# cavelandiah/BBMap

Hardware: AMD Instinct MI355X
Metric: aligned_reads_per_sec (higher is better)
Workload: dtype int32

## Files before the change

bbmap_amd/csrc/mapper.hip:

```cpp
#include <hip/hip_runtime.h>

#include "index_common.h"
#include "mapper_dev.h"

namespace bbmapper {

template <bool KARG> __device__ __forceinline__ const Dev &dev_of(const Dev &byValue) {
    if (KARG) return *(const Dev *)__builtin_amdgcn_kernarg_segment_ptr();
    return byValue;
}

__device__ inline int imin(int a, int b) { return a < b ? a : b; }
__device__ inline int imax(int a, int b) { return a > b ? a : b; }
__device__ inline int iabsdif(int a, int b) { return a > b ? a - b : b - a; }
__device__ inline int max_quality(const Settings &S, int len) { return S.ptsMatch + (len - 1) * S.ptsMatch2; }
__device__ inline int max_imperfect(const Settings &S, int len) { return max_quality(S, len) + S.impDelta; }

__device__ void fix_gaps2(Site &ss) {
    int ra[BBMSA_MAX_GAPS / 2], rb[BBMSA_MAX_GAPS / 2];
    bool alive[BBMSA_MAX_GAPS / 2];
    const int nr = ss.ngaps / 2;
    for (int i = 0; i < nr; i++) { ra[i] = ss.gaps[2 * i]; rb[i] = ss.gaps[2 * i + 1]; alive[i] = true; }
    for (int i = 1; i < nr; i++)
        if (alive[i - 1] && ra[i] - rb[i - 1] <= MINGAP) { ra[i] = imin(ra[i - 1], ra[i]); rb[i] = imax(rb[i - 1], rb[i]); alive[i - 1] = false; }
// ... 728 lines not shown
        }
    }
    const unsigned long long m = __ballot(stillActive);
    if (m) {
        const int lane = threadIdx.x & 63;
        unsigned base = 0;
        if (lane == __builtin_ctzll(m)) base = atomicAdd(&D.counters[CNT_NEXT_ACTIVE], (unsigned)__builtin_popcountll(m));
        base = __shfl(base, __builtin_ctzll(m));
        if (stillActive) D.activeOut[base + __builtin_popcountll(m & ((1ull << lane) - 1ull))] = (int)r;
    }
}

__global__ __launch_bounds__(128) void finish_kernel(const Dev D) {
    const long long r = (long long)blockIdx.x * blockDim.x + threadIdx.x;
    if (r >= D.nreads) return;
    int n = D.mcount[r];
    if (n <= 0) return;
    Site *s = D.ms + r * D.cap;
    n = merge_duplicate_sites(s, n);
    if (!D.S.paired) sort_sites<false>(s, n);
    D.mcount[r] = n;
}

__global__ __launch_bounds__(128) void rescue_plan_kernel(const Dev D) {
    const long long p = (long long)blockIdx.x * blockDim.x + threadIdx.x;
    if (2 * p + 1 >= D.nreads) return;
    PairResc pr = D.pres[p];
    pr.first = 0; pr.count = 0; pr.ran = 0;
    const long long ra = 2 * p + D.pass, rl = 2 * p + (1 - D.pass);
    int na = D.mcount[ra], nl = D.mcount[rl];
    if (na < 0 || nl < 0) { D.pres[p] = pr; return; }
    Site *sa = D.ms + ra * D.cap;
    const Site *sl = D.ms + rl * D.cap;
    int unpairedA;
    if (D.pass == 0) {
        int u1 = 0, u2 = 0;
        for (int i = 0; i < na; i++) if (sa[i].pairedScore == 0) u1++;
        for (int i = 0; i < nl; i++) if (sl[i].pairedScore == 0) u2++;
        pr.unpaired2 = u2; unpairedA = u1;
    } else unpairedA = pr.unpaired2;
    if (!(unpairedA > 0 && na > 0)) { D.pres[p] = pr; return; }
    pr.ran = 1;
    const int lenA = D.reads[ra].len, L = D.reads[rl].len;
    sort_sites<false>(sa, na);
    na = remove_low_quality_paired(sa, na, max_quality(D.S, lenA), D.S.ratioPreRescue, D.S.ratioPreRescue);
    D.mcount[ra] = na;
    const int searchDist = imin(D.S.maxPairDist, 2 * D.S.averagePairDist + 100);
    if (D.S.rescueSkip || searchDist > D.S.maxRescueDist || na == 0) { D.pres[p] = pr; return; }
    const int maxLooseSw = max_quality(D.S, L), maxAnchorSw = max_quality(D.S, lenA), maxImp = max_imperfect(D.S, L);
    const int bestLoose = nl == 0 ? 0 : sl[0].slowScore, bestAnchor = sa[0].slowScore;
    if (bestLoose == maxLooseSw && bestAnchor == maxAnchorSw && sa[0].pairedScore > 0) { D.pres[p] = pr; return; }
    const int rescueScoreLimit = (int)__fmul_rn(0.95f, (float)bestAnchor);
    pr.retainLimit = imax((int)__fmul_rn(0.68f, (float)bestLoose), (int)__fmul_rn(0.4f, (float)maxLooseSw));
    pr.retainLimit2 = imax((int)__fmul_rn(0.95f, (float)bestLoose), (int)__fmul_rn(0.55f, (float)maxLooseSw));
    pr.maxMismatches = bestLoose > maxImp ? 5 : imin(D.S.maxRescueMismatches, (int)__fsub_rn(__fmul_rn(0.60f, (float)L), 1.0f));
    pr.findTip = (D.S.tipSearchDist > 0 && bestLoose < maxImp) ? 1 : 0;
    int cnt = 0;
    for (int i = 0; i < na; i++) { if (sa[i].slowScore < rescueScoreLimit) break; if (sa[i].pairedScore == 0 && !sa[i].rescued) cnt++; }
    if (cnt == 0) { D.pres[p] = pr; return; }
    const unsigned first = atomicAdd(&D.counters[CNT_RESCUE_SEARCHES], (unsigned)cnt);
    pr.first = (int)first; pr.count = cnt;
    if ((long long)first + cnt <= D.rescCap) {
        const bbidx_read rrl = D.reads[rl];
        int k = 0;
        for (int i = 0; i < na; i++) {
            const Site &ssa = sa[i];
            if (ssa.slowScore < rescueScoreLimit) break;
            if (!(ssa.pairedScore == 0 && !ssa.rescued)) continue;
            const int searchIntoAnchor = ssa.stop - ssa.start - 1 + (lenA * 11 / 16);
            const int strand = ssa.strand ^ 1;
            bbresc_job j;
            j.read_off = rrl.bases_off + (strand ? D.minusDelta : 0);
            j.read_len = L; j.chrom = ssa.chrom;
            if (ssa.strand == 0) { j.loc = ssa.stop - searchIntoAnchor; j.idealStart = ssa.stop + D.S.averagePairDist; }
            else { j.loc = ssa.start + searchIntoAnchor; j.idealStart = ssa.start - D.S.averagePairDist; }
            j.searchDist = searchDist + searchIntoAnchor; j.maxAllowedMismatches = pr.maxMismatches;
            j.flags = strand == 1 ? 1 : 0; j.reserved = 0;
            D.rjobs[first + k] = j;
            RescInfo ri; ri.pair = (int)p; ri.anchorSite = i; ri.strand = strand; ri.job = -1;
            D.rinfo[first + k] = ri;
            k++;
        }
    }
    D.pres[p] = pr;
}

template <bool KARG> __global__ __launch_bounds__(128, 5) void rescue_prep_kernel(const Dev Darg) {
    const Dev &D = dev_of<KARG>(Darg);
    const long long p = (long long)blockIdx.x * blockDim.x + threadIdx.x;
    if (2 * p + 1 >= D.nreads) return;
    const PairResc pr = D.pres[p];
    if (pr.count == 0 || (long long)pr.first + pr.count > D.rescCap) return;
    const long long rl = 2 * p + (1 - D.pass);
    const bbidx_read rrl = D.reads[rl];
    const int L = rrl.len, maxImp = max_imperfect(D.S, L), maxScore = max_quality(D.S, L);
    int seq = D.slow[rl].seq;
    for (int k = 0; k < pr.count; k++) {
        const long long q = pr.first + k;
        RescInfo ri = D.rinfo[q];
        const bbresc_result res = D.rres[q];
        const bbresc_job rj = D.rjobs[q];
        Site ss;
        ss.chrom = rj.chrom; ss.strand = ri.strand; ss.start = res.start; ss.stop = res.stop; ss.hits = 0;
        ss.quickScore = ss.score = res.score; ss.slowScore = 0; ss.pairedScore = 0;
        ss.perfect = res.perfect; ss.semiperfect = res.semiperfect; ss.rescued = 1; ss.ngaps = 0;
        for (int i = 0; i < BBMSA_MAX_GAPS; i++) ss.gaps[i] = 0;
        ss.match_job = -1; ss.reserved[0] = 0; ss.reserved[1] = 0;
        ri.job = -1;
        const int reflen = D.chromArrLen[rj.chrom];
        if (res.found == 1 && ss.start >= 0 && ss.stop <= reflen - 1 && res.mismatches <= pr.maxMismatches) {
            const uint8_t *bases = D.bases + rj.read_off;
            const uint8_t *ref = D.chromArr[rj.chrom];
            int sw = score_no_indels(D.S, bases, L, ref, reflen, ss.start);
            if (sw < maxImp && D.S.maxIndel > 0) {
                set_slow_score(ss, sw);
                if (pr.findTip && find_tip_deletions(D.S, ss, bases, L, ref, reflen, maxImp, true, true)) sw = score_no_indels(D.S, bases, L, ref, reflen, ss.start);
                const int minMsaLimit = -D.S.clearzone1e + (int)__fmul_rn(D.S.ratioPaired, (float)maxScore);
                ri.job = emit_fill(D, rl, rrl, ss, -1, D.S.slowRescuePadding, imax(sw, minMsaLimit), 2, seq++);
                atomicAdd(&D.counters[CNT_RESCUE_FILLS], 1u);
                ss.reserved[0] = 2; ss.reserved[1] = sw;
            } else {
                set_slow_score(ss, sw); ss.score = ss.slowScore; set_stop(ss, ss.start + L - 1);
                ss.reserved[0] = 1; ss.reserved[1] = sw;
            }
        }
        D.rsite[q] = ss;
        D.rinfo[q] = ri;
    }
    D.slow[rl].seq = seq;
}

__global__ __launch_bounds__(128) void rescue_finish_kernel(const Dev D) {
    const long long p = (long long)blockIdx.x * blockDim.x + threadIdx.x;
    if (2 * p + 1 >= D.nreads) return;
    const PairResc pr = D.pres[p];
    if (!pr.ran) return;
    const long long ra = 2 * p + D.pass, rl = 2 * p + (1 - D.pass);
    Site *sa = D.ms + ra * D.cap, *sl = D.ms + rl * D.cap;
    int nl = D.mcount[rl];
    const int nsearch = ((long long)pr.first + pr.count > D.rescCap) ? 0 : pr.count;
    const bbidx_read rrl = D.reads[rl];
    const int L = rrl.len, maxScore = max_quality(D.S, L);
    bool overflow = false;
    for (int k = 0; k < nsearch; k++) {
        const long long q = pr.first + k;
        Site ss = D.rsite[q];
        if (ss.reserved[0] == 0) continue;
        const RescInfo ri = D.rinfo[q];
        const uint8_t *bases = D.bases + D.rjobs[q].read_off;
        const uint8_t *ref = D.chromArr[ss.chrom]; const int reflen = D.chromArrLen[ss.chrom];
        if (ss.reserved[0] == 2) {
            const bbmsa_result &res = fill_result(D, ri.job);
            if (res.score_len > 0) { set_slow_score(ss, res.score[0]); ss.score = ss.slowScore; set_start(ss, res.score[1]); set_stop(ss, res.score[2]); ss.match_job = ri.job; }
            else { const int oldStart = D.rres[q].start; set_slow_score(ss, ss.reserved[1]); ss.score = ss.slowScore; set_start(ss, oldStart); set_stop(ss, ss.start + L - 1); }
        }
        ss.reserved[0] = ss.reserved[1] = 0;
        ss.pairedScore = ss.score + 1;
        ss.perfect = (ss.slowScore == maxScore);
        if (ss.perfect) ss.semiperfect = 1; else set_perfect(D.S, ss, bases, L, ref, reflen);
        if (ss.score > pr.retainLimit && ss.start >= 0 && ss.stop <= reflen - 1) {
// ... 162 lines not shown
```

bbmap_amd/csrc/mapper_ctx.h:

```cpp
#pragma once
#include <hip/hip_runtime.h>

#include <cstdio>
#include <thread>
#include <vector>

#include "bbmap_amd.h"
#include "host_common.h"
#include "index_ctx.h"
#include "mapper_dev.h"
#include "msa_ctx.h"

enum { HIO_READS, HIO_BASES, HIO_SCORES, HIO_KEYINFO, HIO_COUNTS, HIO_OFFSETS, HIO_PACKED, BUF_PACK_TMP, BUF_SAM_TMP, BUF_SAM_TEXT, BUF_COUNT };

enum { ACC_STATS, ACC_COV, ACC_HIST, ACC_SPLIT, ACC_COUNT };
struct Accum { bool counted = false; hipStream_t stream = nullptr; };

struct bbmap_ctx {
    bbmap_config cfg;
    bbidx_ctx *index;
    hipStream_t hostStream = nullptr;
    bbidx_launch probeLs;
    bbmsa_ctx *msa, *msaGapped;
    bbmapper::Settings S;
// ... 6 lines not shown
    unsigned *d_counters;
    bbmsa_job *d_jobs; bbmap_jobinfo *d_jinfo; bbmsa_result *d_results; uint8_t *d_match;
    bbmsa_job *d_gjobs; bbmsa_gaps *d_ggaps; bbmap_jobinfo *d_ginfo; bbmsa_result *d_gresults; uint8_t *d_gmatch;
    bbresc_job *d_rjobs; bbmapper::RescInfo *d_rinfo; bbresc_result *d_rres; bbmapper::PairResc *d_pres; bbmap_msite *d_rsite;
    const uint8_t *const *d_chromArr; const int *d_chromArrLen; const uint8_t *refsBase;
    int *d_chromMin;
    long long *d_chromOff;
    long long jobCap, gjobCap, rescCap;
    bbmapper::FinalRead *d_fin; bbmap_final *d_final; uint8_t *d_pool; long long poolUnits, poolUsed, finalFills;
    int matchStride, gmatchStride, maxRows, plainColumns;
    unsigned *h_counters;
    hipEvent_t ev[bbmapper::EV_COUNT];
    bbmap_stats stats;
    long long nJobs, nGapped;
    bool ran;
    bbmap_ctx *tier;
    bool ownsMsa;
    long long narrowMinJobs;
    bool sortWide;
    bool sortPlain;
    bool classSwap;
    bool classOrder;
    bool kernargDev;
    int *d_tierUnits; bbidx_read *d_tierReads; int *d_tierReadIds;
    long long tierReads;
    hipStream_t tierStream;
    hipStream_t dpStream; hipEvent_t evFork, evJoin;
    std::thread tierThread;
    bool tierStarted;
    int tierRc; char tierErr[320];
    long long overAfterBegin;
    struct BatchArgs { int64_t n_reads; const bbidx_read *reads; uint8_t *bases; int64_t minus_delta; const int8_t *baseScores; const int32_t *keyinfo; } batch;
    DevBuf buf[BUF_COUNT];
    bbmap_scafrec *d_scafRec = nullptr;
    int *d_scafTier = nullptr;
    bbmap_samrec *d_samRec = nullptr;
    bbmap_samtags *d_samTags = nullptr;
    int *d_samCounts = nullptr;
    long long *d_samOffsets = nullptr;
    float *d_mapqMax = nullptr;
    long long samTextBytes = 0;
    unsigned long long *d_runStats = nullptr, *d_insertHist = nullptr;
    int adaptive = 0;
    long long numMatedSeen = 0;
    const bbmap_truth *truthNext = nullptr;
    struct CovState *cov = nullptr;
// ... 45 lines not shown
```

bbmap_amd/csrc/mapper_dev.h:

```cpp
#pragma once
#include <hip/hip_runtime.h>

#include "batch_view.h"
#include "bbmap_amd.h"
#include "scaffold.h"

namespace bbmapper {

typedef bbmap_msite Site;

constexpr int GAPBUFFER2 = 128, GAPLEN = 128, MINGAP = 256;
constexpr int TIP_MAX_TIPLEN = 8, OUTER_DIST_MULT = 14, OUTER_DIST_DIV = 32;
constexpr int MIN_TRIM_SINGLE = 3, MIN_TRIM_PAIRED = 2;
constexpr int GAPPED_BIT = 1 << 30;
constexpr int DEAD_MARK = 0x7fffffff;

struct Settings {
    float minRatio, ratioPaired, ratioPreRescue;
    int slowAlignPadding, slowRescuePadding, extraPadding, tipSearchDist, maxPairDist, averagePairDist, maxRescueDist,
        maxRescueMismatches, maxTrimSitesToRetain, trimList, doRescue, alignColumns, clearzone3, maxIndel, expLimit, paired;
    int rescueSkip;
    int ptsMatch, ptsMatch2, ptsSub, ptsSub2, ptsSub3, impDelta, clearzone1e;
    int msaMaxColumns;
    int finalStage;
    int ptsSubR, ptsIns, ptsIns2, ptsIns3, ptsIns4, ptsDel, ptsDel2, ptsDel3, ptsDel4, ptsDel5, ptsGap;
    int finalPolicy, czP, cz1, cz1b, cz1c, czLimit1e;
    int chunkLoads;
};

struct SlowState {
    int idx;
    int phase;
    int minMsaLimit;
    int pending;
    int oldJob;
    int expectedLen;
    int minscore;
    int seq;
};

struct PairResc {
    int first, count;
    int maxMismatches, retainLimit, retainLimit2, findTip;
    int unpaired2;
    int ran;
};

struct RescInfo { int pair, anchorSite, strand, job; };

enum {
    CNT_FILLS = 0,
    CNT_GAPPED_FILLS = 1,
    CNT_NEXT_ACTIVE = 2,
    CNT_OVERFLOWED = 3,
    CNT_RESCUE_SEARCHES = 4,
    CNT_NO_SITE = 5,
    CNT_REFILLS = 6,
    CNT_RESCUE_FILLS = 7,
    CNT_FILLS_DROPPED = 8,
    CNT_CROSS_SCAFFOLD = 9,
    CNT_CLASS_LONG = 10,
    CNT_CLASS_SHORT = 11,
    CNT_TIER_FOUND = 16,
    CNT_TIER_RESOLVED = 17,
    CNT_POOL_UNITS = 20,
    CNT_POOL_AT_FAILURE = 21,
    CNT_POOL_FAILED = 22,
    CNT_LOCAL_READS = 24,
    CNT_LOCAL_UNITS = 25,
    CNT_STAGE_FILLS = 32, CNT_STAGE_GAPPED = 33,
    CNT_STAGE_POOL = 34,
    CNT_WORDS = 64
};
enum { EV_START, EV_PROBE_END, EV_BEGIN_END, EV_SCORE_END, EV_SLOW_END, EV_FINISH_END, EV_RESCUE_END, EV_FINAL_END,
       EV_QUICK_BEGIN, EV_QUICK_END, EV_TIER_BEGIN, EV_TIER_END, EV_COUNT };

struct Dev {
    Settings S;
    const bbidx_read *reads;
    const uint8_t *bases;
    long long minusDelta, nreads;
    const uint8_t *const *chromArr;
    const int *chromArrLen;
    const uint8_t *refsBase;
    const bbidx_site *psites; const int *pnsites; int maxSites;
    Site *ms; int *mcount; int cap;
    int *nearArr;
    SlowState *slow;
    const int *activeIn; int *activeOut; int nActiveIn;
    int *classList;
    int classSwap;
    unsigned *counters;
    bbmsa_job *jobs; bbmap_jobinfo *jinfo; const bbmsa_result *results; long long jobCap;
    bbmsa_job *gjobs; bbmsa_gaps *ggaps; bbmap_jobinfo *ginfo; const bbmsa_result *gresults; long long gjobCap;
    bbresc_job *rjobs; RescInfo *rinfo; const bbresc_result *rres; PairResc *pres; long long rescCap;
    Site *rsite;
    int pass;
    int plainColumns;
    int fillAhead;
    struct FinalRead *fin; bbmap_final *finalOut;
    uint8_t *pool; long long poolUnits;
    const uint8_t *match, *gmatch; int matchStride, gmatchStride;
    bbscaf::Table scaf;
};

struct FinalRead {
    int mapped, paired, ambiguous, perfect, rescued;
    int chrom, strand, start, stop, mapScore;
    int match;
    int matchLen;
    int pc;
    int i;
    int best, scoreChanged, sorting, topObj_, pairedLost;
    int oldSlow, oldScoreS;
    int oldScoreG, gstep;
    int recur, padding, forbidIndels, fixXY, minValid;
    int scoreNoIndel, minLoc, maxLoc, old0, epl, epr, fillKind, minscore, pending, haveMax, cols3;
    int seq;
    int needLocal;
    int reservedI;
// ... 25 lines not shown
```

bbmap_amd/csrc/mapper_host.hip:

```cpp
#include <hip/hip_runtime.h>

#include <algorithm>
#include <cstdlib>
#include <cstring>
#include <new>
#include <thread>
#include <vector>

#include "mapper_ctx.h"

using namespace bbmapper;

extern "C" int bbmap_default_config_profile(int32_t profile, bbmap_config *c) {
    if (!c || (profile != BBIDX_PROFILE_BBMAP && profile != BBIDX_PROFILE_PACBIO)) return bbfail(BBMAP_E_ARG, "bbmap_default_config: bad argument");
    memset(c, 0, sizeof *c);
    c->paired = 0; c->max_reads = 0; c->max_sites = 32;
    c->extraPadding = 10; c->maxPairDist = 32000; c->averagePairDist = 100; c->maxRescueDist = 1200; c->maxRescueMismatches = 32;
    c->maxTrimSitesToRetain = 800; c->trimList = 1; c->doRescue = 1; c->clearzone3 = 800; c->fastCols = 0; c->jobsPerRead = 0;
    c->finalStage = profile == BBIDX_PROFILE_BBMAP ? 1 : 0;
    if (profile == BBIDX_PROFILE_PACBIO) {
        c->max_read_len = 6016; c->minRatio = 0.46f; c->slowAlignPadding = 8; c->slowRescuePadding = 16; c->tipSearchDist = 15;
        c->alignColumns = 7600; c->msaMaxColumns = 7600;
    } else {
        c->max_read_len = 150; c->minRatio = 0.56f; c->slowAlignPadding = 4; c->slowRescuePadding = 8; c->tipSearchDist = 100;
// ... 96 lines not shown
    } else {
        mc.maxColumns = cfg->fastCols > 0 ? cfg->fastCols : 256;
        if (mc.maxColumns > cfg->msaMaxColumns) mc.maxColumns = cfg->msaMaxColumns;
        c->plainColumns = mc.maxColumns;
        gc = mc;
        gc.maxColumns = cfg->msaMaxColumns;
        gc.reserved[0] = 32; gc.reserved[1] = 640 < gc.maxColumns ? 640 : gc.maxColumns;
        if (const char *e = getenv("BBMAP_G2_LANES")) { if (*e) gc.reserved[0] = atoi(e); }
        if (const char *e = getenv("BBMAP_G2_COLS")) { if (*e) gc.reserved[1] = atoi(e) < gc.maxColumns ? atoi(e) : gc.maxColumns; }
        (void)parent;
        c->ownsMsa = true;
        if ((rc = bbmsa_create(&mc, &c->msa)) != BBMAP_OK) return bail(rc);
        if ((rc = bbmsa_create(&gc, &c->msaGapped)) != BBMAP_OK) return bail(rc);
    }
    const long long n = cfg->max_reads;
    const int cap = cfg->max_sites;
    c->narrowMinJobs = getenv("BBMAP_NARROW_MIN_JOBS") ? atoll(getenv("BBMAP_NARROW_MIN_JOBS")) : 32768;
    c->sortWide = !(getenv("BBMAP_SORT_WIDE") && atoi(getenv("BBMAP_SORT_WIDE")) == 0);
    c->sortPlain = !(getenv("BBMAP_SORT_PLAIN") && atoi(getenv("BBMAP_SORT_PLAIN")) == 0);
    c->classOrder = !(getenv("BBMAP_CLASS_ORDER") && atoi(getenv("BBMAP_CLASS_ORDER")) == 0);
    c->classSwap = getenv("BBMAP_CLASS_ORDER") && atoi(getenv("BBMAP_CLASS_ORDER")) == 2;
    c->kernargDev = !(getenv("BBMAP_KERNARG_DEV") && atoi(getenv("BBMAP_KERNARG_DEV")) == 0);
    S.chunkLoads = !(getenv("BBMAP_CHUNK_LOADS") && atoi(getenv("BBMAP_CHUNK_LOADS")) == 0);
    if (!pacbio) {
        const bool wideUnl = !(getenv("BBMAP_WIDE_UNLIMITED") && atoi(getenv("BBMAP_WIDE_UNLIMITED")) == 0);
        bbmsa_set_wide_unlimited(c->msa, wideUnl);
        if (c->msaGapped != c->msa) bbmsa_set_wide_unlimited(c->msaGapped, wideUnl);
    }
    if (!pacbio) {
        const long long lat = getenv("BBMAP_LATENCY_JOBS") ? atoll(getenv("BBMAP_LATENCY_JOBS")) : 4096;
        if ((rc = bbmsa_set_latency_jobs(c->msa, lat)) != BBMAP_OK) return bail(rc);
        if (c->msaGapped != c->msa && (rc = bbmsa_set_latency_jobs(c->msaGapped, lat)) != BBMAP_OK) return bail(rc);
    }
    const int jpr = cfg->jobsPerRead > 0 ? cfg->jobsPerRead : 3;
    c->jobCap = n * jpr + 1024;
    c->gjobCap = parent ? n * 16 + 4096 : (n * jpr) / 24 + 4096;
    if (cfg->jobsPerRead < 0) c->jobCap = c->gjobCap = -(long long)cfg->jobsPerRead;
    c->rescCap = parent ? n * 64 + 1024 : n * 2 + 1024;
    c->matchStride = ((maxRows + c->plainColumns + 15) / 16) * 16;
    c->gmatchStride = ((maxRows + gc.maxColumns + 2 + 128 * 8 + 15) / 16) * 16;
#define DA(ptr, count) if ((rc = dalloc(c, &(ptr), (size_t)(count))) != BBMAP_OK) return bail(rc)
    DA(c->d_psites, n * cap); DA(c->d_pnsites, n);
    DA(c->d_ms, n * cap); DA(c->d_mcount, n); DA(c->d_near, n);
    DA(c->d_slow, n);
    DA(c->d_active[0], n); DA(c->d_active[1], n);
    c->d_classList = nullptr;
    if (c->classOrder) DA(c->d_classList, 2 * n);
    DA(c->d_counters, CNT_WORDS);
    DA(c->d_jobs, c->jobCap); DA(c->d_jinfo, c->jobCap); DA(c->d_results, c->jobCap); DA(c->d_match, c->jobCap * c->matchStride);
    DA(c->d_gjobs, c->gjobCap); DA(c->d_ggaps, c->gjobCap); DA(c->d_ginfo, c->gjobCap); DA(c->d_gresults, c->gjobCap); DA(c->d_gmatch, c->gjobCap * c->gmatchStride);
    DA(c->d_rjobs, c->rescCap); DA(c->d_rinfo, c->rescCap); DA(c->d_rres, c->rescCap); DA(c->d_rsite, c->rescCap);
    DA(c->d_pres, n / 2 + 1);
    if (S.finalStage) {
        c->poolUnits = (n * (long long)(3 * (cfg->max_read_len + 16)) + 65536) / 4;
        if (const char *e = getenv("BBMAP_FINAL_POOL_UNITS")) { if (*e && atoll(e) >= 64) c->poolUnits = atoll(e); }
        DA(c->d_fin, n); DA(c->d_final, n); DA(c->d_pool, c->poolUnits * 4);
    }
    const int nch = index->dev.nchroms;
    DA(c->d_chromMin, nch + 1); DA(c->d_chromOff, nch + 1);
#undef DA
    c->d_chromArr = index->dev.chromArr; c->d_chromArrLen = index->dev.chromArrLen;
// ... 203 lines not shown
    add_dp_ms(c, R.ranPlain, R.ranGapped);
    BBHIP(hipMemsetAsync(c->d_counters + CNT_LOCAL_READS, 0, 8, stream));
    BBTRY(launch<128>(final_end_kernel, units, stream, D));
    BBTRY(read_counters(c, stream));
    finalLocal = h[CNT_LOCAL_READS];
    const long long used = h[CNT_POOL_UNITS], local = h[CNT_LOCAL_UNITS];
    if (used + local + 64 > c->poolUnits) BBTRY(grow_pool(c, stream, D, used, used + local + 65536, false));
    BBTRY(launch<128>(final_local_kernel, units, stream, D));
    return BBMAP_OK;
}


static void fill_dev(bbmap_ctx *c, Dev &D, int64_t n_reads, const bbidx_read *reads, uint8_t *bases, int64_t minus_delta) {
    memset(&D, 0, sizeof D);
    D.S = c->S; D.reads = reads; D.bases = bases; D.minusDelta = minus_delta; D.nreads = n_reads;
    D.chromArr = c->d_chromArr; D.chromArrLen = c->d_chromArrLen; D.refsBase = c->refsBase;
    D.psites = c->d_psites; D.pnsites = c->d_pnsites; D.maxSites = c->cfg.max_sites;
    D.ms = c->d_ms; D.mcount = c->d_mcount; D.cap = c->cfg.max_sites; D.nearArr = c->d_near; D.slow = c->d_slow;
    D.classList = c->d_classList; D.classSwap = c->classSwap ? 1 : 0;
    D.counters = c->d_counters; D.plainColumns = c->plainColumns; D.fillAhead = c->cfg.reserved[0] ? 0 : 1;
    D.jobs = c->d_jobs; D.jinfo = c->d_jinfo; D.results = c->d_results; D.jobCap = c->jobCap;
    D.gjobs = c->d_gjobs; D.ggaps = c->d_ggaps; D.ginfo = c->d_ginfo; D.gresults = c->d_gresults; D.gjobCap = c->gjobCap;
    D.rjobs = c->d_rjobs; D.rinfo = c->d_rinfo; D.rres = c->d_rres; D.pres = c->d_pres; D.rescCap = c->rescCap; D.rsite = c->d_rsite;
    if (c->index->scafFilter) D.scaf = c->index->scaf;
}

static int finish_stats(bbmap_ctx *c, hipStream_t stream, bool whole, long long fillsBefore, long long finalRounds, long long finalLocal) {
    BBHIP(hipEventRecord(c->ev[EV_FINAL_END], stream));
    BBTRY(read_counters(c, stream));
    const unsigned *h = c->h_counters;
    const hipEvent_t *ev = c->ev;
    c->poolUsed = 4ll * h[CNT_POOL_UNITS];
    c->nJobs = h[CNT_FILLS]; c->nGapped = h[CNT_GAPPED_FILLS];
    c->finalFills = c->S.finalStage ? (c->nJobs + c->nGapped) - fillsBefore : 0;
    bbmap_stats &st = c->stats;
    st.fills = c->nJobs; st.gapped_fills = c->nGapped;
    (void)hipEventElapsedTime(&st.ms_final, ev[EV_RESCUE_END], ev[EV_FINAL_END]);
    if (whole) {
        st.reads_overflowed = h[CNT_OVERFLOWED]; st.reads_without_site = h[CNT_NO_SITE];
        st.refills = h[CNT_REFILLS]; st.rescue_fills = h[CNT_RESCUE_FILLS]; st.fills_dropped = h[CNT_FILLS_DROPPED];
        st.sites_cross_scaffold = h[CNT_CROSS_SCAFFOLD];
        (void)hipEventElapsedTime(&st.ms_probe, ev[EV_START], ev[EV_PROBE_END]);
        (void)hipEventElapsedTime(&st.ms_begin, ev[EV_PROBE_END], ev[EV_BEGIN_END]);
        (void)hipEventElapsedTime(&st.ms_score, ev[EV_BEGIN_END], ev[EV_SCORE_END]);
        (void)hipEventElapsedTime(&st.ms_slow, ev[EV_SCORE_END], ev[EV_SLOW_END]);
        (void)hipEventElapsedTime(&st.ms_finish, ev[EV_SLOW_END], ev[EV_FINISH_END]);
// ... 20 lines not shown
    BBTRY(launch<128>(begin_kernel, units, stream, D));
    if (c->tier) {
        BBTRY(launch<128>(collect_overflow_kernel, units, stream, c->d_mcount, units, c->cfg.paired, c->d_tierUnits, c->d_counters + CNT_TIER_FOUND));
    }
    BBHIP(hipEventRecord(c->ev[EV_BEGIN_END], stream));
    BBTRY(launch<128>(DEV_KERNEL(c, score_kernel), n_reads, stream, D));
    BBHIP(hipEventRecord(c->ev[EV_SCORE_END], stream));
    Rounds R; R.finalStage = false; R.jobBase = R.gBase = 0; R.nActive = n_reads;
    for (int round = 0; R.nActive > 0 && round < 4 * c->cfg.max_sites + 4; round++) {
        BBTRY(round_begin(c, stream, D, R, slow_round_kernel));
        if (round == 0) {
            float pms = 0; long long ps[5];
            if (writeRc && bbidx_last_stats_with(c->index, &c->probeLs, (int64_t *)ps, &pms) == BBMAP_OK) for (int i = 0; i < 5; i++) c->stats.probe_stats[i] = ps[i];
            c->overAfterBegin = c->h_counters[CNT_OVERFLOWED];
            if (c->tier && c->h_counters[CNT_TIER_FOUND] > 0 && c->tier->msa != c->msa) tier_start_async(c, c->h_counters[CNT_TIER_FOUND]);
        }
        BBTRY(round_end(c, stream, D, R, bases));
        c->stats.rounds++;
    }
    long long jobBase = R.jobBase, gBase = R.gBase;
    BBHIP(hipEventRecord(c->ev[EV_SLOW_END], stream));
    BBTRY(launch<128>(finish_kernel, n_reads, stream, D));
    BBHIP(hipEventRecord(c->ev[EV_FINISH_END], stream));
    if (c->cfg.paired && c->cfg.doRescue) {
        const long long pairs = n_reads / 2;
        for (int pass = 0; pass < 2; pass++) {
            D.pass = pass;
            BBHIP(hipMemsetAsync(c->d_counters + CNT_RESCUE_SEARCHES, 0, 4, stream));
            BBTRY(launch<128>(rescue_plan_kernel, pairs, stream, D));
            BBTRY(read_counters(c, stream));
            const long long nsearch = c->h_counters[CNT_RESCUE_SEARCHES];
            if (nsearch > c->rescCap) return bbfail(BBMAP_E_NOMEM, "bbmap_map_batch_device: rescue list full");
            c->stats.rescue_scans += nsearch;
            if (nsearch == 0) {
                BBTRY(launch<128>(rescue_finish_kernel, pairs, stream, D));
                continue;
            }
            hipEvent_t q0 = c->ev[EV_QUICK_BEGIN], q1 = c->ev[EV_QUICK_END];
            BBHIP(hipEventRecord(q0, stream));
            BBTRY(bbpipe_quick_rescue_device(stream, nsearch, c->d_rjobs, bases, (const int64_t *)c->d_chromOff, c->d_chromArrLen, c->d_chromMin, c->refsBase,
                                            c->d_rres, c->S.ptsMatch, c->S.ptsMatch2, 1, 100));
            BBHIP(hipEventRecord(q1, stream));
            if (jobBase + nsearch > c->jobCap || gBase + nsearch > c->gjobCap) BBTRY(grow_logs(c, stream, D, jobBase + nsearch, gBase + nsearch, jobBase, gBase));
            BBTRY(launch<128>(DEV_KERNEL(c, rescue_prep_kernel), pairs, stream, D));
            BBTRY(read_counters(c, stream));
            { float ms = 0; if (hipEventElapsedTime(&ms, q0, q1) == hipSuccess) c->stats.ms_quick_rescue += ms; }
            const long long total = c->h_counters[CNT_FILLS], gtotal = c->h_counters[CNT_GAPPED_FILLS];
            if (total > c->jobCap || gtotal > c->gjobCap) return bbfail(BBMAP_E_HIP, "bbmap_map_batch_device: rescue fills beyond the reserved log entries (internal error)");
            BBTRY(run_fills(c, stream, bases, jobBase, total - jobBase, gBase, gtotal - gBase));
            const bool ranPlain = total > jobBase, ranGapped = gtotal > gBase;
            jobBase = total; gBase = gtotal;
            BBTRY(launch<128>(rescue_finish_kernel, pairs, stream, D));
            BBHIP(hipStreamSynchronize(stream));
            add_dp_ms(c, ranPlain, ranGapped);
        }
    }
    BBHIP(hipEventRecord(c->ev[EV_RESCUE_END], stream));
    c->finalFills = 0; c->poolUsed = 0;
    long long finalRounds = 0, finalLocal = 0;
    if (c->S.finalStage) BBTRY(run_final_stage(c, stream, D, n_reads, bases, jobBase, gBase, finalRounds, finalLocal));
    BBTRY(finish_stats(c, stream, true, jobBase + gBase, finalRounds, finalLocal));
    c->ran = true;
    return BBMAP_OK;
}

static int tier_pass(bbmap_ctx *c, hipStream_t s, long long found) {
    bbmap_ctx *t = c->tier;
    const bbmap_ctx::BatchArgs &B = c->batch;
    const int paired = c->cfg.paired;
    c->tierReads = 0; t->ran = false;
    std::vector<int> ids((size_t)found);
    BBHIP(hipMemcpyAsync(ids.data(), c->d_tierUnits, 4 * (size_t)found, hipMemcpyDeviceToHost, s));
    BBHIP(hipStreamSynchronize(s));
    std::sort(ids.begin(), ids.end());
    const long long room = paired ? t->cfg.max_reads / 2 : t->cfg.max_reads;
    const long long take = found < room ? found : room;
    BBHIP(hipMemcpyAsync(c->d_tierUnits, ids.data(), 4 * (size_t)take, hipMemcpyHostToDevice, s));
    BBTRY(launch<128>(gather_reads_kernel, take, s, B.reads, c->d_tierUnits, (int)take, paired, c->d_tierReads, c->d_tierReadIds));
    BBHIP(hipStreamSynchronize(s));
    const long long tn = paired ? 2 * take : take;
    BBTRY(map_records(t, s, tn, c->d_tierReads, B.bases, B.minus_delta, B.baseScores, B.keyinfo, false));
    c->tierReads = tn;
    return BBMAP_OK;
}
// ... 4 lines not shown
        int rc = hipSetDevice(c->cfg.device) == hipSuccess ? BBMAP_OK : BBMAP_E_HIP;
        if (rc == BBMAP_OK) rc = tier_pass(c, c->tierStream, found);
        if (rc != BBMAP_OK) { snprintf(c->tierErr, sizeof c->tierErr, "overflow tier: %s", bbmap_last_error()); }
        c->tierRc = rc;
    });
}

static int tier_finish(bbmap_ctx *c, hipStream_t stream) {
    bbmap_ctx *t = c->tier;
    const long long tn = c->tierReads;
    if (tn == 0) return BBMAP_OK;
    BBHIP(hipMemsetAsync(c->d_counters + CNT_TIER_RESOLVED, 0, 4, stream));
    BBTRY(launch<128>(mark_tier_kernel, tn, stream, c->d_mcount, t->d_mcount, c->d_tierReadIds, (int)tn, c->d_counters + CNT_TIER_RESOLVED));
    BBTRY(read_counters(c, stream));
    bbmap_stats &st = c->stats; const bbmap_stats &ts = t->stats;
    st.reads_reprobed = tn;
    st.reads_overflowed -= (long long)c->h_counters[CNT_TIER_RESOLVED];
    st.reads_without_site += ts.reads_without_site;
    st.fills += ts.fills; st.gapped_fills += ts.gapped_fills; st.refills += ts.refills; st.rescue_scans += ts.rescue_scans;
    st.rescue_fills += ts.rescue_fills; st.fills_dropped += ts.fills_dropped;
    st.final_fills += ts.final_fills; st.final_local += ts.final_local;
    st.dp_narrow_launches += ts.dp_narrow_launches; st.dp_sorted_launches += ts.dp_sorted_launches;
    st.sites_cross_scaffold += ts.sites_cross_scaffold;
    if (getenv("BBMAP_TIER_DEBUG"))
        fprintf(stderr, "[bbmap tier] reads %lld: probe %.2f begin %.2f score %.2f slow %.2f (rounds %lld) finish %.2f rescue %.2f total %.2f\n",
                tn, ts.ms_probe, ts.ms_begin, ts.ms_score, ts.ms_slow, (long long)ts.rounds, ts.ms_finish, ts.ms_rescue, ts.ms_total);
    return BBMAP_OK;
}

static int rescue_skip_rule(bbmap_ctx *c, bool *skip) {
    *skip = false;
    if (!c->d_runStats) return BBMAP_OK;
    bbmap_runstats rs;
    BBHIP(hipStreamSynchronize(c->accum[ACC_STATS].stream));
    BBHIP(hipMemcpy(&rs, c->d_runStats, sizeof rs, hipMemcpyDeviceToHost));
    *skip = rs.mappedRetained2 > 1000 && rs.numMated * 20LL < rs.mappedRetained2;
    return BBMAP_OK;
}

static int adapt_after_batch(bbmap_ctx *c, hipStream_t stream) {
    if (!(c->adaptive & BBMAP_ADAPT_INSERT_LENGTH)) return BBMAP_OK;
    bbmap_runstats rs;
    BBHIP(hipMemcpyAsync(&rs, c->d_runStats, sizeof rs, hipMemcpyDeviceToHost, stream));
    BBHIP(hipStreamSynchronize(stream));
    const bool heldPaired = rs.numMated > c->numMatedSeen;
    c->numMatedSeen = rs.numMated;
// ... 101 lines not shown
```

bbmap_amd/csrc/mapper_output.hip:

```cpp
#include <hip/hip_runtime.h>

#include <cstdint>
#include <cstring>
#include <initializer_list>
#include <memory>
#include <vector>

#include "coverage.h"
#include "mapper_ctx.h"
#include "read_hist.h"
#include "ref_split.h"
#include "run_stats.h"
#include "sam_records.h"
#include "scan_offsets.h"

using namespace bbmapper;

extern "C" int bbmap_pack_sites_device(bbmap_ctx *c, void *stream_, int64_t n_reads, int32_t *counts, int64_t *offsets, bbmap_msite *packed,
                                       int64_t packed_cap) {
    if (!c || !counts || !offsets || !packed) return bbfail(BBMAP_E_ARG, "bbmap_pack_sites_device: null argument");
    if (!c->ran || n_reads != c->stats.reads) return bbfail(BBMAP_E_ARG, "bbmap_pack_sites_device: n_reads is not the last batch's");
    hipStream_t stream = (hipStream_t)stream_;
    BBHIP(hipSetDevice(c->cfg.device));
    const long long n = n_reads;
// ... 766 lines not shown
    SplitState *v = c->split;
    if (!v) return BBMAP_OK;
    return reset_state(c, ACC_SPLIT, {{v->state.p, (size_t)bbpipe_refsplit_state_bytes(v->cfg.nkeys, v->cfg.nsets)}});
}

extern "C" int bbidx_get_chrom_table(bbidx_ctx *ix, int32_t *nchroms, const uint8_t **chromArr, int32_t *chromArrLen, int32_t cap) {
    if (!ix || !nchroms) return bbfail(BBMAP_E_ARG, "bbidx_get_chrom_table: null argument");
    *nchroms = ix->dev.nchroms;
    if (!chromArr && !chromArrLen) return BBMAP_OK;
    if (cap < ix->dev.nchroms + 1) return bbfail(BBMAP_E_ARG, "bbidx_get_chrom_table: buffers too small (need nchroms + 1 entries)");
    BBHIP(hipSetDevice(ix->device));
    if (chromArr) BBHIP(hipMemcpy(chromArr, ix->dev.chromArr, sizeof(void *) * (size_t)(ix->dev.nchroms + 1), hipMemcpyDeviceToHost));
    if (chromArrLen) BBHIP(hipMemcpy(chromArrLen, ix->dev.chromArrLen, 4 * (size_t)(ix->dev.nchroms + 1), hipMemcpyDeviceToHost));
    return BBMAP_OK;
}

extern "C" int bbmap_last_stats(bbmap_ctx *c, bbmap_stats *out) {
    if (!c || !out) return bbfail(BBMAP_E_ARG, "bbmap_last_stats: null argument");
    if (!c->ran) return bbfail(BBMAP_E_ARG, "bbmap_last_stats: no batch has been mapped yet");
    *out = c->stats;
    return BBMAP_OK;
}

extern "C" int bbmap_copy_to_host(void *dst, const void *src_device, int64_t bytes) {
    if (bytes < 0 || (bytes > 0 && (!dst || !src_device))) return bbfail(BBMAP_E_ARG, "bbmap_copy_to_host: bad argument");
    if (bytes > 0) BBHIP(hipMemcpy(dst, src_device, (size_t)bytes, hipMemcpyDeviceToHost));
    return BBMAP_OK;
}
```

bbmap_amd/mapper.py:

```python
import ctypes as C

import numpy as np
import torch

from . import _lib
from . import msa as M
from .index import READ_DTYPE, read_lens

MSITE_DTYPE = np.dtype([("chrom", "<i4"), ("strand", "<i4"), ("start", "<i4"), ("stop", "<i4"), ("hits", "<i4"),
                        ("quickScore", "<i4"), ("score", "<i4"), ("slowScore", "<i4"), ("pairedScore", "<i4"),
                        ("perfect", "<i4"), ("semiperfect", "<i4"), ("rescued", "<i4"), ("ngaps", "<i4"),
                        ("gaps", "<i4", (16,)), ("match_job", "<i4"), ("reserved", "<i4", (2,))])
JOBINFO_DTYPE = np.dtype([("read", "<i4"), ("seq", "<i4"), ("kind", "<i4"), ("site", "<i4")])
FINAL_DTYPE = np.dtype([("mapped", "<i4"), ("chrom", "<i4"), ("strand", "<i4"), ("start", "<i4"), ("stop", "<i4"), ("mapScore", "<i4"),
                        ("paired", "<i4"), ("ambiguous", "<i4"), ("perfect", "<i4"), ("rescued", "<i4"), ("match_len", "<i4"),
                        ("nsites", "<i4"), ("match_off", "<i8"), ("reserved", "<i4", (2,))])
SCAFREC_DTYPE = np.dtype([("scaffold", "<i4"), ("start", "<i4"), ("stop", "<i4"), ("pos", "<i4"), ("end", "<i4"), ("scaflen", "<i4"),
                          ("flags", "<i4"), ("reserved", "<i4")])
SCAF_MAPPED, SCAF_PAIRED, SCAF_INBOUNDS, SCAF_SAME_SCAFFOLD = 1, 2, 4, 8
SAMREC_DTYPE = np.dtype([("flag", "<i4"), ("mapq", "<i4"), ("rname", "<i4"), ("rnext", "<i4"), ("pos", "<i4"), ("pnext", "<i4"),
                         ("tlen", "<i4"), ("nm", "<i4"), ("am", "<i4"), ("tags", "<i4"), ("cigar_off", "<i8"), ("cigar_len", "<i4"),
                         ("md_len", "<i4"), ("md_off", "<i8")])
SAM_CIGAR13, SAM_MD = 1, 2
SAM_TAG_XT = 1
# ... 366 lines not shown
                          [b[:w.nbins] for b in bins] if binsize > 0 else None, self.di.scaffold_names)

    def reset_coverage(self):
        _lib.check(self.L.bbmap_reset_coverage(self.h), "bbmap_reset_coverage")

    def pack_sites(self, counts, offsets, packed):
        stream = torch.cuda.current_stream().cuda_stream
        assert counts.numel() == self.n + 1 and offsets.numel() == self.n + 1 and packed.numel() % MSITE_DTYPE.itemsize == 0
        _lib.check(self.L.bbmap_pack_sites_device(self.h, C.c_void_p(stream), self.n, counts.data_ptr(), offsets.data_ptr(),
                                                  packed.data_ptr(), packed.numel() // MSITE_DTYPE.itemsize), "bbmap_pack_sites_device")

    def output_pointers(self):
        o = bbmap_output()
        _lib.check(self.L.bbmap_get_output(self.h, C.byref(o)), "bbmap_get_output")
        return o

    def stats(self):
        st = bbmap_stats()
        _lib.check(self.L.bbmap_last_stats(self.h, C.byref(st)), "bbmap_last_stats")
        d = {n: getattr(st, n) for n, _ in bbmap_stats._fields_ if n not in ("probe_stats",)}
        d["probe_stats"] = list(st.probe_stats)
        return d

    def _fetch_output(self, o, n, with_match, rows=None):
        cap = o.cap
        out = dict(cap=cap)
        ns = n if rows is None else min(rows, n)
        rec = lambda p, count, dt: _copy(p, count * dt.itemsize, self.dev).view(dt)
        out["sites"] = rec(o.sites, ns * cap, MSITE_DTYPE).reshape(ns, cap)
        out["nsites"] = _copy(o.nsites, n * 4, self.dev).view(np.int32)
        nj, ng = int(o.n_jobs), int(o.n_gapped_jobs)
        out["jobs"] = rec(o.jobs, nj, M.JOB_DTYPE)
        out["results"] = rec(o.results, nj, M.RESULT_DTYPE)
        out["jobinfo"] = rec(o.jobinfo, nj, JOBINFO_DTYPE)
        out["gjobs"] = rec(o.gjobs, ng, M.JOB_DTYPE)
        out["gresults"] = rec(o.gresults, ng, M.RESULT_DTYPE)
        out["gjobinfo"] = rec(o.gjobinfo, ng, JOBINFO_DTYPE)
        out["ggaps"] = rec(o.ggaps, ng, M.GAPS_DTYPE)
        out["match_stride"], out["gmatch_stride"] = o.match_stride, o.gmatch_stride
        if with_match:
            out["match"] = _copy(o.match, nj * o.match_stride, self.dev).reshape(nj, o.match_stride)
            out["gmatch"] = _copy(o.gmatch, ng * o.gmatch_stride, self.dev).reshape(ng, o.gmatch_stride)
        return out

    def fetch(self, with_match=True, rows=None):
        o = bbmap_output()
# ... 72 lines not shown
```

include/bbmap_amd.h:

```cpp
#ifndef BBMAP_AMD_H
#define BBMAP_AMD_H

#include <stdint.h>

#ifdef __cplusplus
extern "C" {
#endif

#define BBMAP_AMD_ABI_VERSION 6

enum {
    BBMAP_OK = 0,
    BBMAP_E_NODEVICE = -1,
    BBMAP_E_ARG = -2,
    BBMAP_E_NOMEM = -3,
    BBMAP_E_HIP = -4,
    BBMAP_E_SHAPE = -5
};

const char *bbmap_last_error(void);
int bbmap_abi_version(void);


enum {
// ... 532 lines not shown
    int32_t xs;
    int32_t nh, sm, xm;
    int32_t ys;
    int32_t yl_query, yl_ref;
    int32_t yi_good, yi_bad;
    int32_t yi_perfect;
    int32_t yr;
    int32_t x8;
    int32_t xb;
    int32_t introns;
    int32_t splices;
} bbmap_samtags;
int bbmap_get_sam_records_cfg(bbmap_ctx *ctx, void *stream, const bbmap_sam_config *cfg, const bbmap_samrec **recs,
                              const bbmap_samtags **tags, const uint8_t **text, int64_t *text_bytes);
int bbmap_get_sam_cfg(bbmap_ctx *ctx, int64_t n_reads, const bbmap_sam_config *cfg, bbmap_samrec *out, bbmap_samtags *tags_out,
                      uint8_t *text_out, int64_t text_cap, int64_t *text_bytes);
int64_t bbpipe_sam_records_workspace_bytes(int64_t n_reads, int32_t max_read_len);
int bbpipe_sam_records_device(void *stream, int64_t n_reads, int32_t paired, const bbmap_sam_config *cfg, int32_t max_read_len,
                              const bbidx_read *reads, const uint8_t *bases, const bbmap_final *finals, const uint8_t *pool,
                              const bbmap_scafrec *scaf, const bbmap_msite *sites, const int32_t *nsites, int32_t cap,
                              const uint8_t *const *chrom_arr, const int32_t *chrom_arr_len, bbmap_samrec *recs, bbmap_samtags *tags,
                              uint8_t *text, int64_t text_cap, int64_t *text_bytes_dev, void *workspace, int64_t workspace_bytes);
int bbmap_last_stats(bbmap_ctx *ctx, bbmap_stats *out);

enum { BBMAP_INSERT_HIST_BINS = 40001 };
enum { BBMAP_RUNSTATS_MAX_WAVES = 8192 };
typedef struct bbmap_runstats {
    int64_t mappedRetained1;
    int64_t mappedRetainedBases1;
    int64_t ambiguousBestAlignment1;
    int64_t ambiguousBestAlignmentBases1;
    int64_t matchCountM1;
    int64_t matchCountS1;
    int64_t matchCountD1;
    int64_t matchCountI1;
    int64_t matchCountN1;
    int64_t readCountS1;
    int64_t readCountD1;
    int64_t readCountI1;
    int64_t readCountN1;
    int64_t readCountE1;
    int64_t rescuedP1;
    int64_t rescuedM1;
    int64_t perfectMatch1;
    int64_t perfectMatchBases1;
    int64_t perfectHitCount1;
// ... 246 lines not shown
```

Before: 10.46 million.

## Plan both rescue directions in the first pass when direction 0 needs no searches

The rescue planner now takes a per-pair direction. In pass 0, a pair whose direction 0 produces no rescue searches immediately plans direction 1, after merging duplicate sites on the mate. Pass 1 then skips pairs already handled, which moves work from the second pass into the first and can leave the second pass with few or no searches. It also adds optional split counters and an API to report them, and doubles the rescue capacity, which costs memory and adds a behavioural risk if the merge timing changes results.

```diff
diff --git a/bbmap_amd/csrc/mapper.hip b/bbmap_amd/csrc/mapper.hip
--- a/bbmap_amd/csrc/mapper.hip
+++ b/bbmap_amd/csrc/mapper.hip
@@ -774,34 +774,31 @@
     D.mcount[r] = n;
 }
 
-__global__ __launch_bounds__(128) void rescue_plan_kernel(const Dev D) {
-    const long long p = (long long)blockIdx.x * blockDim.x + threadIdx.x;
-    if (2 * p + 1 >= D.nreads) return;
-    PairResc pr = D.pres[p];
+__device__ bool rescue_plan_direction(const Dev &D, long long p, PairResc &pr) {
     pr.first = 0; pr.count = 0; pr.ran = 0;
-    const long long ra = 2 * p + D.pass, rl = 2 * p + (1 - D.pass);
+    const long long ra = 2 * p + pr.dir, rl = 2 * p + (1 - pr.dir);
     int na = D.mcount[ra], nl = D.mcount[rl];
-    if (na < 0 || nl < 0) { D.pres[p] = pr; return; }
+    if (na < 0 || nl < 0) return false;
     Site *sa = D.ms + ra * D.cap;
     const Site *sl = D.ms + rl * D.cap;
     int unpairedA;
-    if (D.pass == 0) {
+    if (pr.dir == 0) {
         int u1 = 0, u2 = 0;
         for (int i = 0; i < na; i++) if (sa[i].pairedScore == 0) u1++;
         for (int i = 0; i < nl; i++) if (sl[i].pairedScore == 0) u2++;
         pr.unpaired2 = u2; unpairedA = u1;
     } else unpairedA = pr.unpaired2;
-    if (!(unpairedA > 0 && na > 0)) { D.pres[p] = pr; return; }
+    if (!(unpairedA > 0 && na > 0)) return true;
     pr.ran = 1;
     const int lenA = D.reads[ra].len, L = D.reads[rl].len;
     sort_sites<false>(sa, na);
     na = remove_low_quality_paired(sa, na, max_quality(D.S, lenA), D.S.ratioPreRescue, D.S.ratioPreRescue);
     D.mcount[ra] = na;
     const int searchDist = imin(D.S.maxPairDist, 2 * D.S.averagePairDist + 100);
-    if (D.S.rescueSkip || searchDist > D.S.maxRescueDist || na == 0) { D.pres[p] = pr; return; }
+    if (D.S.rescueSkip || searchDist > D.S.maxRescueDist || na == 0) return true;
     const int maxLooseSw = max_quality(D.S, L), maxAnchorSw = max_quality(D.S, lenA), maxImp = max_imperfect(D.S, L);
     const int bestLoose = nl == 0 ? 0 : sl[0].slowScore, bestAnchor = sa[0].slowScore;
-    if (bestLoose == maxLooseSw && bestAnchor == maxAnchorSw && sa[0].pairedScore > 0) { D.pres[p] = pr; return; }
+    if (bestLoose == maxLooseSw && bestAnchor == maxAnchorSw && sa[0].pairedScore > 0) return true;
     const int rescueScoreLimit = (int)__fmul_rn(0.95f, (float)bestAnchor);
     pr.retainLimit = imax((int)__fmul_rn(0.68f, (float)bestLoose), (int)__fmul_rn(0.4f, (float)maxLooseSw));
     pr.retainLimit2 = imax((int)__fmul_rn(0.95f, (float)bestLoose), (int)__fmul_rn(0.55f, (float)maxLooseSw));
@@ -809,7 +806,7 @@
     pr.findTip = (D.S.tipSearchDist > 0 && bestLoose < maxImp) ? 1 : 0;
     int cnt = 0;
     for (int i = 0; i < na; i++) { if (sa[i].slowScore < rescueScoreLimit) break; if (sa[i].pairedScore == 0 && !sa[i].rescued) cnt++; }
-    if (cnt == 0) { D.pres[p] = pr; return; }
+    if (cnt == 0) return true;
     const unsigned first = atomicAdd(&D.counters[CNT_RESCUE_SEARCHES], (unsigned)cnt);
     pr.first = (int)first; pr.count = cnt;
     if ((long long)first + cnt <= D.rescCap) {
@@ -834,6 +831,40 @@
             k++;
         }
     }
+    return true;
+}
+
+__device__ void rescue_count_split(const Dev &D, int c0, int c1) {
+    if (c0 > 0 && c1 > 0) {
+        atomicAdd(&D.counters[CNT_SPLIT_PAIRS_BOTH], 1u);
+        atomicAdd(&D.counters[CNT_SPLIT_SCANS_BOTH_D0], (unsigned)c0); atomicAdd(&D.counters[CNT_SPLIT_SCANS_BOTH_D1], (unsigned)c1);
+    } else if (c0 > 0) { atomicAdd(&D.counters[CNT_SPLIT_PAIRS_D0], 1u); atomicAdd(&D.counters[CNT_SPLIT_SCANS_D0], (unsigned)c0); }
+    else if (c1 > 0) { atomicAdd(&D.counters[CNT_SPLIT_PAIRS_D1], 1u); atomicAdd(&D.counters[CNT_SPLIT_SCANS_D1], (unsigned)c1); }
+}
+
+__global__ __launch_bounds__(128) void rescue_plan_kernel(const Dev D) {
+    const long long p = (long long)blockIdx.x * blockDim.x + threadIdx.x;
+    if (2 * p + 1 >= D.nreads) return;
+    PairResc pr = D.pres[p];
+    if (D.pass == 0) {
+        pr.dir = 0; pr.again = 1;
+        const bool whole = rescue_plan_direction(D, p, pr);
+        if (D.rescueMerge && whole && pr.count == 0) {
+            if (pr.ran) {
+                const long long rl = 2 * p + 1;
+                D.mcount[rl] = merge_duplicate_sites(D.ms + rl * D.cap, D.mcount[rl]);
+            }
+            pr.dir = 1; pr.again = 0;
+            rescue_plan_direction(D, p, pr);
+            if (D.rescueCounts) rescue_count_split(D, 0, pr.count);
+        }
+    } else {
+        const int c0 = pr.dir == 0 ? pr.count : 0;
+        if (D.rescueMerge && !pr.again) { pr.first = 0; pr.count = 0; pr.ran = 0; D.pres[p] = pr; return; }
+        pr.dir = 1; pr.again = 0;
+        rescue_plan_direction(D, p, pr);
+        if (D.rescueCounts) rescue_count_split(D, c0, pr.count);
+    }
     D.pres[p] = pr;
 }
 
@@ -843,7 +874,7 @@
     if (2 * p + 1 >= D.nreads) return;
     const PairResc pr = D.pres[p];
     if (pr.count == 0 || (long long)pr.first + pr.count > D.rescCap) return;
-    const long long rl = 2 * p + (1 - D.pass);
+    const long long rl = 2 * p + (1 - pr.dir);
     const bbidx_read rrl = D.reads[rl];
     const int L = rrl.len, maxImp = max_imperfect(D.S, L), maxScore = max_quality(D.S, L);
     int seq = D.slow[rl].seq;
@@ -887,7 +918,7 @@
     if (2 * p + 1 >= D.nreads) return;
     const PairResc pr = D.pres[p];
     if (!pr.ran) return;
-    const long long ra = 2 * p + D.pass, rl = 2 * p + (1 - D.pass);
+    const long long ra = 2 * p + pr.dir, rl = 2 * p + (1 - pr.dir);
     Site *sa = D.ms + ra * D.cap, *sl = D.ms + rl * D.cap;
     int nl = D.mcount[rl];
     const int nsearch = ((long long)pr.first + pr.count > D.rescCap) ? 0 : pr.count;
diff --git a/bbmap_amd/csrc/mapper_ctx.h b/bbmap_amd/csrc/mapper_ctx.h
--- a/bbmap_amd/csrc/mapper_ctx.h
+++ b/bbmap_amd/csrc/mapper_ctx.h
@@ -52,6 +52,9 @@
     bool classSwap;
     bool classOrder;
     bool kernargDev;
+    bool rescueMerge;
+    bool rescueCounts;
+    long long rescSplit[8];
     int *d_tierUnits; bbidx_read *d_tierReads; int *d_tierReadIds;
     long long tierReads;
     hipStream_t tierStream;
diff --git a/bbmap_amd/csrc/mapper_dev.h b/bbmap_amd/csrc/mapper_dev.h
--- a/bbmap_amd/csrc/mapper_dev.h
+++ b/bbmap_amd/csrc/mapper_dev.h
@@ -44,6 +44,8 @@
     int maxMismatches, retainLimit, retainLimit2, findTip;
     int unpaired2;
     int ran;
+    int dir;
+    int again;
 };
 
 struct RescInfo { int pair, anchorSite, strand, job; };
@@ -70,6 +72,8 @@
     CNT_LOCAL_UNITS = 25,
     CNT_STAGE_FILLS = 32, CNT_STAGE_GAPPED = 33,
     CNT_STAGE_POOL = 34,
+    CNT_SPLIT_PAIRS_D0 = 40, CNT_SPLIT_PAIRS_D1 = 41, CNT_SPLIT_PAIRS_BOTH = 42,
+    CNT_SPLIT_SCANS_D0 = 43, CNT_SPLIT_SCANS_D1 = 44, CNT_SPLIT_SCANS_BOTH_D0 = 45, CNT_SPLIT_SCANS_BOTH_D1 = 46,
     CNT_WORDS = 64
 };
 enum { EV_START, EV_PROBE_END, EV_BEGIN_END, EV_SCORE_END, EV_SLOW_END, EV_FINISH_END, EV_RESCUE_END, EV_FINAL_END,
@@ -96,6 +100,8 @@
     bbresc_job *rjobs; RescInfo *rinfo; const bbresc_result *rres; PairResc *pres; long long rescCap;
     Site *rsite;
     int pass;
+    int rescueMerge;
+    int rescueCounts;
     int plainColumns;
     int fillAhead;
     struct FinalRead *fin; bbmap_final *finalOut;
diff --git a/bbmap_amd/csrc/mapper_host.hip b/bbmap_amd/csrc/mapper_host.hip
--- a/bbmap_amd/csrc/mapper_host.hip
+++ b/bbmap_amd/csrc/mapper_host.hip
@@ -142,6 +142,8 @@
     c->classSwap = getenv("BBMAP_CLASS_ORDER") && atoi(getenv("BBMAP_CLASS_ORDER")) == 2;
     c->kernargDev = !(getenv("BBMAP_KERNARG_DEV") && atoi(getenv("BBMAP_KERNARG_DEV")) == 0);
     S.chunkLoads = !(getenv("BBMAP_CHUNK_LOADS") && atoi(getenv("BBMAP_CHUNK_LOADS")) == 0);
+    c->rescueMerge = !(getenv("BBMAP_RESCUE_MERGE") && atoi(getenv("BBMAP_RESCUE_MERGE")) == 0);
+    c->rescueCounts = getenv("BBMAP_RESCUE_COUNTS") && atoi(getenv("BBMAP_RESCUE_COUNTS")) != 0;
     if (!pacbio) {
         const bool wideUnl = !(getenv("BBMAP_WIDE_UNLIMITED") && atoi(getenv("BBMAP_WIDE_UNLIMITED")) == 0);
         bbmsa_set_wide_unlimited(c->msa, wideUnl);
@@ -157,6 +159,7 @@
     c->gjobCap = parent ? n * 16 + 4096 : (n * jpr) / 24 + 4096;
     if (cfg->jobsPerRead < 0) c->jobCap = c->gjobCap = -(long long)cfg->jobsPerRead;
     c->rescCap = parent ? n * 64 + 1024 : n * 2 + 1024;
+    if (c->rescueMerge) c->rescCap *= 2;
     c->matchStride = ((maxRows + c->plainColumns + 15) / 16) * 16;
     c->gmatchStride = ((maxRows + gc.maxColumns + 2 + 128 * 8 + 15) / 16) * 16;
 #define DA(ptr, count) if ((rc = dalloc(c, &(ptr), (size_t)(count))) != BBMAP_OK) return bail(rc)
@@ -406,6 +409,7 @@
     D.jobs = c->d_jobs; D.jinfo = c->d_jinfo; D.results = c->d_results; D.jobCap = c->jobCap;
     D.gjobs = c->d_gjobs; D.ggaps = c->d_ggaps; D.ginfo = c->d_ginfo; D.gresults = c->d_gresults; D.gjobCap = c->gjobCap;
     D.rjobs = c->d_rjobs; D.rinfo = c->d_rinfo; D.rres = c->d_rres; D.pres = c->d_pres; D.rescCap = c->rescCap; D.rsite = c->d_rsite;
+    D.rescueMerge = c->rescueMerge ? 1 : 0; D.rescueCounts = c->rescueCounts ? 1 : 0;
     if (c->index->scafFilter) D.scaf = c->index->scaf;
 }
 
@@ -472,6 +476,7 @@
     BBHIP(hipEventRecord(c->ev[EV_SLOW_END], stream));
     BBTRY(launch<128>(finish_kernel, n_reads, stream, D));
     BBHIP(hipEventRecord(c->ev[EV_FINISH_END], stream));
+    for (long long &v : c->rescSplit) v = 0;
     if (c->cfg.paired && c->cfg.doRescue) {
         const long long pairs = n_reads / 2;
         for (int pass = 0; pass < 2; pass++) {
@@ -482,6 +487,7 @@
             const long long nsearch = c->h_counters[CNT_RESCUE_SEARCHES];
             if (nsearch > c->rescCap) return bbfail(BBMAP_E_NOMEM, "bbmap_map_batch_device: rescue list full");
             c->stats.rescue_scans += nsearch;
+            if (pass == 1) c->rescSplit[7] = nsearch;
             if (nsearch == 0) {
                 BBTRY(launch<128>(rescue_finish_kernel, pairs, stream, D));
                 continue;
@@ -510,6 +516,12 @@
     long long finalRounds = 0, finalLocal = 0;
     if (c->S.finalStage) BBTRY(run_final_stage(c, stream, D, n_reads, bases, jobBase, gBase, finalRounds, finalLocal));
     BBTRY(finish_stats(c, stream, true, jobBase + gBase, finalRounds, finalLocal));
+    for (int i = 0; i < 7; i++) c->rescSplit[i] = c->rescueCounts ? (long long)c->h_counters[CNT_SPLIT_PAIRS_D0 + i] : -1;
+    if (c->rescueCounts) {
+        const long long *s = c->rescSplit;
+        fprintf(stderr, "rescue counts: reads %lld, pairs searching in direction 0 only %lld (%lld searches), in direction 1 only %lld (%lld), "
+                "in both %lld (%lld + %lld); searches of the second pass %lld\n", (long long)n_reads, s[0], s[3], s[1], s[4], s[2], s[5], s[6], s[7]);
+    }
     c->ran = true;
     return BBMAP_OK;
 }
@@ -560,6 +572,7 @@
     st.final_fills += ts.final_fills; st.final_local += ts.final_local;
     st.dp_narrow_launches += ts.dp_narrow_launches; st.dp_sorted_launches += ts.dp_sorted_launches;
     st.sites_cross_scaffold += ts.sites_cross_scaffold;
+    for (int i = 0; i < 8; i++) if (c->rescSplit[i] >= 0 && t->rescSplit[i] >= 0) c->rescSplit[i] += t->rescSplit[i];
     if (getenv("BBMAP_TIER_DEBUG"))
         fprintf(stderr, "[bbmap tier] reads %lld: probe %.2f begin %.2f score %.2f slow %.2f (rounds %lld) finish %.2f rescue %.2f total %.2f\n",
                 tn, ts.ms_probe, ts.ms_begin, ts.ms_score, ts.ms_slow, (long long)ts.rounds, ts.ms_finish, ts.ms_rescue, ts.ms_total);
diff --git a/bbmap_amd/csrc/mapper_output.hip b/bbmap_amd/csrc/mapper_output.hip
--- a/bbmap_amd/csrc/mapper_output.hip
+++ b/bbmap_amd/csrc/mapper_output.hip
@@ -812,6 +812,13 @@
     return BBMAP_OK;
 }
 
+extern "C" int bbmap_last_rescue_split(bbmap_ctx *c, int64_t *counts8) {
+    if (!c || !counts8) return bbfail(BBMAP_E_ARG, "bbmap_last_rescue_split: null argument");
+    if (!c->ran) return bbfail(BBMAP_E_ARG, "bbmap_last_rescue_split: no batch has been mapped yet");
+    for (int i = 0; i < 8; i++) counts8[i] = c->rescSplit[i];
+    return BBMAP_OK;
+}
+
 extern "C" int bbmap_copy_to_host(void *dst, const void *src_device, int64_t bytes) {
     if (bytes < 0 || (bytes > 0 && (!dst || !src_device))) return bbfail(BBMAP_E_ARG, "bbmap_copy_to_host: bad argument");
     if (bytes > 0) BBHIP(hipMemcpy(dst, src_device, (size_t)bytes, hipMemcpyDeviceToHost));
diff --git a/bbmap_amd/mapper.py b/bbmap_amd/mapper.py
--- a/bbmap_amd/mapper.py
+++ b/bbmap_amd/mapper.py
@@ -412,6 +412,13 @@
         d["probe_stats"] = list(st.probe_stats)
         return d
 
+    def rescue_split(self):
+        c = (C.c_int64 * 8)()
+        _lib.check(self.L.bbmap_last_rescue_split(self.h, c), "bbmap_last_rescue_split")
+        names = ("pairs_dir0_only", "pairs_dir1_only", "pairs_both", "scans_dir0_only", "scans_dir1_only", "scans_both_dir0",
+                 "scans_both_dir1", "scans_second_pass")
+        return {n: int(c[i]) for i, n in enumerate(names)}
+
     def _fetch_output(self, o, n, with_match, rows=None):
         cap = o.cap
         out = dict(cap=cap)
diff --git a/include/bbmap_amd.h b/include/bbmap_amd.h
--- a/include/bbmap_amd.h
+++ b/include/bbmap_amd.h
@@ -578,6 +578,7 @@
                               const uint8_t *const *chrom_arr, const int32_t *chrom_arr_len, bbmap_samrec *recs, bbmap_samtags *tags,
                               uint8_t *text, int64_t text_cap, int64_t *text_bytes_dev, void *workspace, int64_t workspace_bytes);
 int bbmap_last_stats(bbmap_ctx *ctx, bbmap_stats *out);
+int bbmap_last_rescue_split(bbmap_ctx *ctx, int64_t *counts8);
 
 enum { BBMAP_INSERT_HIST_BINS = 40001 };
 enum { BBMAP_RUNSTATS_MAX_WAVES = 8192 };
```

After: 10.47 million, median of 2. About the same (+0.1%).
